# ucas-vg/PointTinyBenchmark

Hardware: AMD Instinct MI355X
Metric: img/s (640x640) CPR R50-FPN fwd+loss (higher is better)
Workload: dtype fp32

## Files before the change

include/cpr_hip.h:

```cpp
#ifndef CPR_HIP_H
#define CPR_HIP_H
#ifdef __cplusplus
extern "C" {
#endif

#define CPR_ERR_ARG (-1001)
#define CPR_ERR_UNSUPPORTED (-1002)

int cpr_version(void);

#define CPR_CONV_RELU 1
#define CPR_CONV_OUT_BF16 2
#define CPR_CONV_RES_MASK 4
#define CPR_CONV_COLSUM 8
int cpr_conv2d_fwd(const float* in, const float* wgt, float* out, const float* scale, const float* bias,
                   const float* residual, const float* in_a, const float* in_b, float* gn_part, int N, int H, int W,
                   int Cin, int Cout, int KH, int KW, int stride, int pad, int Kpad, int flags, int in_relu,
                   int* variant_out, void* stream);
int cpr_conv2d_fwd_dil(const float* in, const float* wgt, float* out, const float* scale, const float* bias,
                       const float* residual, const float* in_a, const float* in_b, float* gn_part, int N, int H, int W,
                       int Cin, int Cout, int KH, int KW, int stride, int pad, int dil, int Kpad, int flags, int in_relu,
                       int* variant_out, void* stream);

int cpr_conv2d_dual_fwd(const float* in, const float* wgt, const float* in2, const float* wgt2, float* out,
// ... 316 lines not shown
int cpr_bn_sync_bwd_merge(const double* records, int R, const double* count, const float* dout, const float* z, const float* y,
                          const float* center, const float* mean, const float* rstd, const float* gamma, float* dy, float* ws, long long M,
                          int C, void* stream);
int cpr_p2p_out_bf16_fwd(const void* x, const float* a, const float* b, const float* w, const float* bias, float* taps, float* out,
                         int N, int H, int W, int Cin, int J, void* stream);
int cpr_p2p_out_bf16_dgrad(const float* dout, int ldd, const float* w, void* dx, int out_bf16, int N, int H, int W, int Cin, int J,
                           void* stream);
int cpr_p2p_out_bf16_wgrad_ws(int N, int H, int W, int Cin, int J);
int cpr_p2p_out_bf16_wgrad(const void* x, const float* a, const float* b, const float* dout, int ldd, float* gw, float* gb, float* ws,
                           int N, int H, int W, int Cin, int J, void* stream);
int cpr_bn_fold_multi(const void* jobs_dev, int n, int max_c, void* stream);
int cpr_pack_weights_multi(const void* jobs_dev, int n, int total_blocks, void* stream);
int cpr_pack_weights_bf16_multi(const void* jobs_dev, int n, int total_blocks, void* stream);
int cpr_p2p_loss_bwd(const float* logits, const float* pred, const long long* gt_inds, const float* gt_pts,
                     const int* gt_labels, const int* gt_start, const float* npos, float* dcls, float* dreg, int B, int M,
                     int C, int Cp, int Rp, float alpha, float gamma, float beta, float pos_w, float neg_w, float reg_norm,
                     float w_cls, float w_reg, float gamma_p, const float* upstream, int cls_mode, int reg_mode, void* stream);
int cpr_p2p_loss_bwd_levels(const float* logits, const float* pred, const long long* gt_inds, const float* gt_pts,
                            const int* gt_labels, const int* gt_start, const float* npos, int B, int M, int C, int P, int L,
                            const int* level_hw, const int* level_off, const int* level_cp, const int* level_rp,
                            float* const* level_dcls, float* const* level_dreg, float alpha, float gamma, float beta, float pos_w,
                            float neg_w, float reg_norm, float w_cls, float w_reg, float gamma_p, const float* upstream,
                            int cls_mode, int reg_mode, void* stream);
int cpr_grad_sumsq(const float* g, long long n, double* ws_partial, double* out, int accumulate, void* stream);
int cpr_sgd_step(float* p, const float* grad, float* buf, const double* norm2, long long n, float lr, float mu, float wd,
                 float max_norm, float grad_scale, int first, void* stream);
int cpr_adam_step(float* p, const float* grad, float* exp_avg, float* exp_avg_sq, const double* norm2, long long n, double lr,
                  double beta1, double beta2, double eps, double wd, float step_size, float bc2_sqrt, float max_norm,
                  float grad_scale, int decoupled, void* stream);

int cpr_preprocess_u8(const unsigned char* img, const int* flip, const float* mean3, const float* stdinv3, int to_rgb,
                      float* out, int N, int H, int W, int Hp, int Wp, void* stream);
int cpr_clip_flip_boxes(float* boxes, const int* img_of, const int* flip, const int* img_hw, int n, int clip,
                        void* stream);

typedef struct cpr_preprocess_job {
    const unsigned char* src;
    long long out_off;
    double scale_x, scale_y;
    int pitch, src_w, src_h, x0, y0, cw, ch, dw, dh, flip, Hp, Wp;
} cpr_preprocess_job;
int cpr_preprocess_jobs_u8(const void* jobs_dev, int n_jobs, const float* mean3, const float* stdinv3, int to_rgb, float* out,
                           long long total_out_pixels, void* stream);
int cpr_scale_clip_flip_boxes(float* boxes, const int* img_of, const int* flip, const int* img_hw, const float* scale4, int n,
                              int clip, void* stream);

#ifdef CPR_BENCH_HOOKS
int cpr_conv_force_tile(int bm, int bn);
int cpr_conv_set_pipeline(int mode);
int cpr_conv_set_stream(int on);
int cpr_conv_set_ablation(int mode);
int cpr_wgrad_set_ablation(int mode);
int cpr_conv_set_extra_lds(int bytes);
int cpr_wino_set_variant(int sched, int ablate);
int cpr_bf16_set_dma(int on);
int cpr_bf16_set_wfrag(int on);
int cpr_wino_set_staging(int var, int tpx);
int cpr_wino32_set_debug(int ablate, int wg_per_cu, int stagger_pct);
int cpr_lsa_phase_clocks(long long* host_out, int reset);
int cpr_bn_set_finalize_only(int on);
#endif

#ifdef __cplusplus
}
#endif
#endif
```

pointtinybenchmark_amd/_lib.py:

```python
import ctypes
import os

_HERE = os.path.dirname(os.path.abspath(__file__))
LIB_PATH = os.path.join(_HERE, 'csrc', 'libcprhip.so')

_p = ctypes.c_void_p
_i = ctypes.c_int
_f = ctypes.c_float
_l = ctypes.c_longlong
_d = ctypes.c_double

SIGNATURES = {
    'cpr_version': [],
    'cpr_conv2d_fwd': [_p, _p, _p, _p, _p, _p, _p, _p, _p, _i, _i, _i, _i, _i, _i, _i, _i, _i, _i, _i, _i, _p, _p],
    'cpr_conv2d_fwd_dil': [_p] * 9 + [_i] * 13 + [_p, _p],
    'cpr_conv2d_dual_fwd': [_p] * 9 + [_i] * 16 + [_p, _p],
    'cpr_conv1x1_stream_fwd': [_p, _p, _p, _p, _p, _p, _l, _i, _i, _i, _p],
    'cpr_conv_wgrad_bf16_workspace_s': [_i] * 9,
    'cpr_conv_wgrad_bf16_s': [_p, _i, _p, _i, _p, _p] + [_i] * 8 + [_p],
    'cpr_wino_pack_weights': [_p, _p, _i, _i, _i, _p],
    'cpr_conv3x3_wino_fwd': [_p, _p, _p, _p, _p, _p, _p, _p, _i, _i, _i, _i, _i, _i, _i, _i, _p],
    'cpr_wino32_pack_weights': [_p, _p, _i, _i, _i, _p],
    'cpr_conv3x3_wino32_slots': [_i, _i],
    'cpr_conv3x3_wino32_fwd': [_p, _p, _p, _p, _p, _p, _p, _p, _i, _i, _i, _i, _i, _i, _i, _i, _p],
# ... 116 lines not shown
    'cpr_res2_conv_wgrad': [_p, _i, _i, _p, _i, _i, _p, _i, _i, _p, _p] + [_i] * 6 + [_p],
    'cpr_res2_pool_fwd': [_p, _i, _i, _p, _i, _i] + [_i] * 5 + [_p],
    'cpr_res2_relu_bwd_colsum': [_p, _i, _i, _p, _i, _i, _p, _i, _i, _p, _p, _l, _i, _p],
    'cpr_res2_pool_bwd': [_p, _i, _i, _p, _i, _i] + [_i] * 5 + [_p],
    'cpr_splat_chunks': [_i] * 3,
    'cpr_splat_gap': [_p, _p, _p] + [_i] * 4 + [_p],
    'cpr_splat_attn': [_p] * 9 + [_i] * 3 + [_p],
    'cpr_splat_apply': [_p] * 3 + [_i] * 5 + [_p],
    'cpr_splat_attn_grad': [_p] * 4 + [_i] * 5 + [_p],
    'cpr_splat_attn_bwd': [_p] * 18 + [_i] * 3 + [_p],
    'cpr_splat_apply_bwd': [_p] * 7 + [_i] * 5 + [_p],
    'cpr_dw3x3_pack': [_p, _p, _p, _i, _p],
    'cpr_dw3x3_fwd': [_p] * 5 + [_i] * 6 + [_p],
    'cpr_dw3x3_dgrad_workspace': [_i] * 4,
    'cpr_dw3x3_dgrad': [_p] * 7 + [_i] * 5 + [_p],
    'cpr_dw3x3_wgrad_workspace': [_i] * 5,
    'cpr_dw3x3_wgrad': [_p] * 4 + [_i] * 7 + [_p],
    'cpr_relu6_bwd_colsum_ws': [_l, _i],
    'cpr_relu6_bwd_colsum': [_p] * 6 + [_l, _i, _p],
    'cpr_clamp6': [_p, _l, _p],
    'cpr_spin': [ctypes.c_longlong, _p],
    'cpr_bn_fold': [_p, _p, _p, _p, _f, _p, _p, _p, _i, _p],
    'cpr_bn_train_ws': [_l, _i],
    'cpr_bn_batch_stats': [_p] * 6 + [_f, _f] + [_p] * 8 + [_l, _i, _p],
    'cpr_bn_apply': [_p] * 10 + [_l, _i, _i, _p],
    'cpr_bn_train_bwd': [_p] * 11 + [_l, _i, _p],
    'cpr_bn_sync_ws': [_l, _i],
    'cpr_bn_sync_stats_local': [_p, _p, _p, _l, _i, _p],
    'cpr_bn_sync_stats_merge': [_p, _i] + [_p] * 6 + [_f, _f] + [_p] * 8 + [_i, _p],
    'cpr_bn_sync_bwd_local': [_p] * 10 + [_l, _i, _p],
    'cpr_bn_sync_bwd_merge': [_p, _i] + [_p] * 10 + [_l, _i, _p],
    'cpr_p2p_out_bf16_fwd': [_p] * 7 + [_i] * 5 + [_p],
    'cpr_p2p_out_bf16_dgrad': [_p, _i, _p, _p] + [_i] * 6 + [_p],
    'cpr_p2p_out_bf16_wgrad_ws': [_i] * 5,
    'cpr_p2p_out_bf16_wgrad': [_p] * 4 + [_i] + [_p] * 3 + [_i] * 5 + [_p],
    'cpr_p2p_loss_bwd': [_p] * 9 + [_i] * 5 + [_f] * 9 + [_p, _i, _i, _p],
    'cpr_p2p_loss_bwd_levels': [_p] * 7 + [_i] * 5 + [_p] * 6 + [_f] * 9 + [_p, _i, _i, _p],
    'cpr_grad_sumsq': [_p, _l, _p, _p, _i, _p],
    'cpr_sgd_step': [_p, _p, _p, _p, _l, _f, _f, _f, _f, _f, _i, _p],
    'cpr_adam_step': [_p, _p, _p, _p, _p, _l, _d, _d, _d, _d, _d, _f, _f, _f, _f, _i, _p],
}

BENCH_SIGNATURES = {
    'cpr_lsa_phase_clocks': [_p, _i],
    'cpr_wino32_set_debug': [_i, _i, _i],
    'cpr_conv_force_tile': [_i, _i],
    'cpr_conv_set_pipeline': [_i],
    'cpr_conv_set_stream': [_i],
    'cpr_conv_set_ablation': [_i],
    'cpr_wgrad_set_ablation': [_i],
    'cpr_wino_set_variant': [_i, _i],
    'cpr_wino_set_staging': [_i, _i],
    'cpr_conv_set_extra_lds': [_i],
    'cpr_bf16_set_dma': [_i],
    'cpr_bf16_set_wfrag': [_i],
    'cpr_bn_set_finalize_only': [_i],
}
BENCH_LIB_PATH = os.path.join(_HERE, 'csrc', 'libcprhip_bench.so')

_lib = None


class CprHipError(RuntimeError):
    pass


def load():
    global _lib
    if _lib is not None:
        return _lib
    path, sigs = LIB_PATH, dict(SIGNATURES)
    if os.environ.get('CPR_BENCH_HOOKS', '0') == '1':
        path = BENCH_LIB_PATH
        sigs.update(BENCH_SIGNATURES)
    if not os.path.exists(path):
        raise CprHipError('%s not found: run `python -m pointtinybenchmark_amd.build%s` (no CPU fallback exists)'
                          % (path, ' --bench-hooks' if path == BENCH_LIB_PATH else ''))
    lib = ctypes.CDLL(path)
    for name, argtypes in sigs.items():
        fn = getattr(lib, name, None)
        if fn is None:
            raise CprHipError('symbol %s missing from %s (stale build?)' % (name, path))
        fn.argtypes = argtypes
        fn.restype = ctypes.c_int
    _lib = lib
    return lib


def call(name, *args, positive=False):
    rc = getattr(load(), name)(*args)
    if positive and rc >= 0:
        return rc
    if rc != 0:
        if rc == -1001:
            raise CprHipError('%s: invalid argument' % name)
        if rc == -1002:
            raise CprHipError('%s: unsupported configuration' % name)
        raise CprHipError('%s failed with hipError %d' % (name, -rc))
    return rc
```

pointtinybenchmark_amd/csrc/conv_mfma.hip:

```cpp
#include <type_traits>
#include "common.h"

struct ConvParams {
    const float* in;
    const float* wgt;
    float* out;
    const float* scale;
    const float* bias;
    const float* residual;
    const float* in_a;
    const float* in_b;
    float* gn_part;
    int N, H, W, Cin, OH, OW, Cout, KH, KW, stride, pad, Kpad, M, relu, in_relu, out_bf16;
    int res_mask;
    int tilesM, tilesN;
    const float* in2;
    const float* wgt2;
    const float* scale2;
    const float* bias2;
    int H2, W2, Cin2, stride2, Kpad2;
    int dil;
};

constexpr int BK = 32;
constexpr int LDSW = 36;

template <int BM, int BN, int MODE, bool XF, int PIPE, int ABL = 0, bool DUAL = false, bool DIL = false>
__global__ __launch_bounds__(256, 2) void conv_mfma_kernel(ConvParams p) {
    static_assert(!DUAL || (MODE == 0 && !XF && PIPE == 1 && ABL == 0), "the dual-source form exists for the plain pipelined instances");
    static_assert(!DIL || (MODE == 0 && !XF && PIPE == 1 && ABL == 0 && !DUAL), "the dilated form exists for the plain pipelined instances");
    constexpr int WM = BM / 2;
    constexpr int WN = BN / 2;
    constexpr int MI = WM / 32;
    constexpr int NI = WN / 32;
    constexpr int AL = BM * 8 / 256;
    constexpr int BL = BN * 8 / 256;
    constexpr int XFMAX = 512;
    __shared__ __attribute__((aligned(16))) float smem[2 * (BM + BN) * LDSW + (XF ? 2 * XFMAX : 0)];
    float* As = smem;
    float* Bs = smem + 2 * BM * LDSW;
    float* ABs = smem + 2 * (BM + BN) * LDSW;

    const int T = p.tilesM * p.tilesN;
    const int per = (T + 7) >> 3;
    const int tile = (blockIdx.x & 7) * per + (blockIdx.x >> 3);
    if (tile >= T) return;
    const int tm = tile / p.tilesN, tn = tile - tm * p.tilesN;
    const int m0 = tm * BM, n0 = tn * BN;

    const int tid = threadIdx.x, lane = tid & 63, wave = tid >> 6;
    const int c4 = tid & 7, r0 = tid >> 3;

    int iy0[AL], ix0[AL], nimg[AL], rowoff[AL];
    bool mok[AL];
    const int ohw = p.OH * p.OW;
    const bool gemm = (p.KH == 1) & (p.KW == 1) & (p.stride == 1) & (p.pad == 0) & (MODE == 0);
#pragma unroll
    for (int j = 0; j < AL; ++j) {
        int m = m0 + r0 + 32 * j;
        mok[j] = m < p.M;
        int mm = mok[j] ? m : 0;
        if (gemm) {
            nimg[j] = 0; iy0[j] = 0; ix0[j] = 0;
            rowoff[j] = mm * p.Cin + c4 * 4;
        } else {
            int n = mm / ohw;
            int rem = mm - n * ohw;
            int oy = rem / p.OW, ox = rem - oy * p.OW;
            nimg[j] = n;
            iy0[j] = oy * p.stride - p.pad;
            ix0[j] = ox * p.stride - p.pad;
            rowoff[j] = ((n * p.H + iy0[j]) * p.W + ix0[j]) * p.Cin + c4 * 4;
        }
    }
    __amdgpu_buffer_rsrc_t rs_in = __builtin_amdgcn_make_buffer_rsrc(
        const_cast<float*>(p.in), 0, (int)((size_t)p.N * p.H * p.W * p.Cin * 4), 0x00020000);
    __amdgpu_buffer_rsrc_t rs_w = __builtin_amdgcn_make_buffer_rsrc(
        const_cast<float*>(p.wgt), 0, (int)((size_t)p.Cout * p.Kpad * 4), 0x00020000);
    int cin_cur = p.Cin;
    bool second = false;
    const float* wrow[BL];
    int woff[BL];
    bool wok[BL];
#pragma unroll
    for (int j = 0; j < BL; ++j) {
        int c = n0 + r0 + 32 * j;
        wok[j] = c < p.Cout;
        wrow[j] = p.wgt + (size_t)(wok[j] ? c : 0) * p.Kpad + c4 * 4;
        woff[j] = wok[j] ? (c * p.Kpad + c4 * 4) * 4 : -1;
    }

    constexpr int NSET = (!XF && BM == 64 && BN == 64) ? 2 : 1;
    f32x4 ra[NSET][AL], rb[NSET][BL], xa, xb;
    unsigned okmask = 0;
    bool any_pad = true;
    int tapoff = 0;
    int kh = 0, kw = 0, c0 = 0;
    constexpr bool xform = XF;
    const float relu_floor = p.in_relu ? 0.f : -INFINITY;
    const int nblk = (m0 < p.M ? m0 : 0) / ohw;
    if (XF) {
        for (int i = tid; i < p.Cin; i += 256) {
            ABs[i] = p.in_a[nblk * p.Cin + i];
            ABs[XFMAX + i] = p.in_b[nblk * p.Cin + i];
        }
        __syncthreads();
    }

    int voffA[AL];
    unsigned okcur = 0;
    auto refresh_rows = [&]() {
        okcur = 0;
        const int dl = DIL ? p.dil : 1;
        const int tapshift = (kh * dl * p.W + kw * dl) * p.Cin;
#pragma unroll
        for (int j = 0; j < AL; ++j) {
            const int iy = iy0[j] + kh * dl, ix = ix0[j] + kw * dl;
            const bool ok = mok[j] & ((unsigned)iy < (unsigned)p.H) & ((unsigned)ix < (unsigned)p.W);
            okcur |= (ok ? 1u : 0u) << j;
            voffA[j] = ok ? (rowoff[j] + tapshift) * 4 : -1;
        }
    };
    if (MODE == 0) refresh_rows();
    auto load_a = [&](auto set_c, int kt, int j) {
        constexpr int SET = decltype(set_c)::value;
        if (MODE == 0) {
            if (j == 0) {
                okmask = okcur;
                tapoff = c0 * 4;
            }
            ra[SET][j] = __builtin_bit_cast(f32x4, __builtin_amdgcn_raw_buffer_load_b128(rs_in, voffA[j], tapoff, 0));
        } else {
            if (j == 0) okmask = 0;
            const int tap = kt * 8 + c4;
            const int th = (p.KW == 7) ? tap / 7 : tap / p.KW;
            const int tw = tap - th * p.KW;
            const int iy = iy0[j] + th, ix = ix0[j] + tw;
            const bool ok = (tap < p.KH * p.KW) & mok[j] & ((unsigned)iy < (unsigned)p.H) & ((unsigned)ix < (unsigned)p.W);
            okmask |= (ok ? 1u : 0u) << j;
            const int voff = ok ? ((nimg[j] * p.H + iy) * p.W + ix) * 16 : -1;
            ra[SET][j] = __builtin_bit_cast(f32x4, __builtin_amdgcn_raw_buffer_load_b128(rs_in, voff, 0, 0));
        }
    };
    auto load_x_advance = [&]() {
        if (MODE == 0) {
            if (xform) {
                xa = *reinterpret_cast<const f32x4*>(ABs + c0 + c4 * 4);
                xb = *reinterpret_cast<const f32x4*>(ABs + XFMAX + c0 + c4 * 4);
            }
            c0 += BK;
            if (c0 == cin_cur) {
                c0 = 0;
                if (!(DUAL && second)) {
                    if (++kw == p.KW) { kw = 0; ++kh; }
                    refresh_rows();
                }
            }
        }
    };
    int kt_last = p.Kpad / BK - 1;
    auto load_b = [&](auto set_c, int kt, int j) {
        constexpr int SET = decltype(set_c)::value;
        rb[SET][j] = __builtin_bit_cast(f32x4, __builtin_amdgcn_raw_buffer_load_b128(rs_w, woff[j], min(kt, kt_last) * (BK * 4), 0));
    };
    auto store_a = [&](auto set_c, int buf, int j) {
        constexpr int SET = decltype(set_c)::value;
        f32x4 v = ra[SET][j];
        if (MODE == 0 && xform) {
            v = v * xa + xb;
            v.x = fmaxf(v.x, relu_floor); v.y = fmaxf(v.y, relu_floor);
            v.z = fmaxf(v.z, relu_floor); v.w = fmaxf(v.w, relu_floor);
        }
        if (MODE == 0 && xform) {
            if (j == 0) any_pad = __builtin_amdgcn_ballot_w64(okmask != ((1u << AL) - 1u)) != 0;
            if (any_pad) {
                if (!((okmask >> j) & 1u)) v = f32x4{0.f, 0.f, 0.f, 0.f};
            }
        }
        *reinterpret_cast<f32x4*>(As + buf * BM * LDSW + (r0 + 32 * j) * LDSW + c4 * 4) = v;
    };
    auto store_b = [&](auto set_c, int buf, int j) {
        constexpr int SET = decltype(set_c)::value;
        *reinterpret_cast<f32x4*>(Bs + buf * BN * LDSW + (r0 + 32 * j) * LDSW + c4 * 4) = rb[SET][j];
    };
    auto load_tile = [&](auto set_c, int kt) {
#pragma unroll
        for (int j = 0; j < AL; ++j) load_a(set_c, kt, j);
        load_x_advance();
#pragma unroll
        for (int j = 0; j < BL; ++j) load_b(set_c, kt, j);
    };
    auto store_tile = [&](auto set_c, int buf) {
#pragma unroll
        for (int j = 0; j < AL; ++j) store_a(set_c, buf, j);
#pragma unroll
        for (int j = 0; j < BL; ++j) store_b(set_c, buf, j);
    };
    using Set0 = std::integral_constant<int, 0>;
    using Set1 = std::integral_constant<int, NSET - 1>;

    f32x16 acc[MI][NI];
#pragma unroll
    for (int i = 0; i < MI; ++i)
#pragma unroll
        for (int j = 0; j < NI; ++j)
#pragma unroll
            for (int r = 0; r < 16; ++r) acc[i][j][r] = 0.f;

    f32x16 acc2[DUAL ? MI : 1][DUAL ? NI : 1];
    if (DUAL) {
#pragma unroll
        for (int i = 0; i < MI; ++i)
#pragma unroll
            for (int j = 0; j < NI; ++j)
#pragma unroll
                for (int r = 0; r < 16; ++r) acc2[DUAL ? i : 0][DUAL ? j : 0][r] = 0.f;
    }

    const int wm = wave & 1, wn = wave >> 1;
    const int arow = wm * WM + (lane & 31);
    const int brow = wn * WN + (lane & 31);
    const int koff = 4 * (lane >> 5);

    int KT = p.Kpad / BK;
    const float* a_lds = As + arow * LDSW + koff;
    const float* b_lds = Bs + brow * LDSW + koff;
    auto read_frags = [&](int buf, int kk, f32x4 (&fa)[MI], f32x4 (&fb)[NI]) {
#pragma unroll
        for (int i = 0; i < MI; ++i)
            fa[i] = *reinterpret_cast<const f32x4*>(a_lds + buf * BM * LDSW + i * 32 * LDSW + kk * 8);
#pragma unroll
        for (int j = 0; j < NI; ++j)
            fb[j] = *reinterpret_cast<const f32x4*>(b_lds + buf * BN * LDSW + j * 32 * LDSW + kk * 8);
    };
    auto mfma_group = [&](const f32x4 (&fa)[MI], const f32x4 (&fb)[NI]) {
#pragma unroll
        for (int t = 0; t < 4; ++t)
#pragma unroll
            for (int i = 0; i < MI; ++i)
#pragma unroll
                for (int j = 0; j < NI; ++j)
                    acc[i][j] = __builtin_amdgcn_mfma_f32_32x32x2f32(fa[i][t], fb[j][t], acc[i][j], 0, 0, 0);
    };

    if (PIPE == 0) {
        load_tile(Set0{}, 0);
        store_tile(Set0{}, 0);
        __syncthreads();
        for (int kt = 0; kt < KT; ++kt) {
            const int buf = kt & 1;
            if (kt + 1 < KT) load_tile(Set0{}, kt + 1);
#pragma unroll
            for (int kk = 0; kk < 4; ++kk) {
                f32x4 fa[MI], fb[NI];
                read_frags(buf, kk, fa, fb);
                mfma_group(fa, fb);
            }
            if (kt + 1 < KT) store_tile(Set0{}, buf ^ 1);
            __syncthreads();
        }
    } else {
      auto kloop = [&](f32x16 (&accX)[MI][NI]) {
        f32x4 fa0[MI], fb0[NI], fa1[MI], fb1[NI];
        load_tile(Set0{}, 0);
        store_tile(Set0{}, 0);
        load_tile(Set1{}, 1);
        if (NSET == 2) load_tile(Set0{}, 2);
        __syncthreads();
        read_frags(0, 0, fa0, fb0);
        constexpr int NM = 4 * MI * NI;
        constexpr int NF = MI + NI;
        constexpr int P1 = NF + AL + BL, P2 = NF + AL + 1 + BL;
        constexpr int PPF = (NF + NM - 1) / NM, PP1 = (P1 + NM - 1) / NM, PP2 = (P2 + NM - 1) / NM;
#define MFMA_SLOT(FA, FB, q)                                                                                  \
    accX[((q) / NI) % MI][(q) % NI] = __builtin_amdgcn_mfma_f32_32x32x2f32(                                 \
        FA[((q) / NI) % MI][(q) / (MI * NI)], FB[(q) % NI][(q) / (MI * NI)], accX[((q) / NI) % MI][(q) % NI], 0, 0, 0)
#define FRAG_PIECE(FA, FB, buf, kk, z)                                                                        \
    do {                                                                                                      \
        if ((z) < MI)                                                                                         \
            FA[(z) < MI ? (z) : 0] = *reinterpret_cast<const f32x4*>(a_lds + (buf) * BM * LDSW +              \
                                                                     ((z) < MI ? (z) : 0) * 32 * LDSW + (kk) * 8); \
        else                                                                                                  \
            FB[(z) >= MI ? (z) - MI : 0] = *reinterpret_cast<const f32x4*>(                                   \
                b_lds + (buf) * BN * LDSW + ((z) >= MI ? (z) - MI : 0) * 32 * LDSW + (kk) * 8);                \
    } while (0)
        auto iteration = [&](auto nxt_c, int kt) {
            const int buf = kt & 1;
#pragma unroll
            for (int q = 0; q < NM; ++q) {
                MFMA_SLOT(fa0, fb0, q);
#pragma unroll
                for (int z = q * PPF; z < (q + 1) * PPF; ++z)
                    if (z < NF && !(ABL & 2)) FRAG_PIECE(fa1, fb1, buf, 1, z);
                __builtin_amdgcn_sched_barrier(0);
            }
#pragma unroll
            for (int q = 0; q < NM; ++q) {
                MFMA_SLOT(fa1, fb1, q);
#pragma unroll
                for (int z = q * PP1; z < (q + 1) * PP1; ++z) {
                    if (z < NF) { if (!(ABL & 2)) FRAG_PIECE(fa0, fb0, buf, 2, z); }
                    else if (ABL & 1) {}
                    else if (ABL & 8) {
                        if (z < NF + AL) asm volatile("" ::"v"(ra[decltype(nxt_c)::value][z - NF < AL ? z - NF : 0]));
                        else if (z < P1) asm volatile("" ::"v"(rb[decltype(nxt_c)::value][z - NF - AL < BL ? z - NF - AL : 0]));
                    }
                    else if (z < NF + AL) store_a(nxt_c, buf ^ 1, z - NF);
                    else if (z < P1) store_b(nxt_c, buf ^ 1, z - NF - AL);
                }
                __builtin_amdgcn_sched_barrier(0);
            }
#pragma unroll
            for (int q = 0; q < NM; ++q) {
                MFMA_SLOT(fa0, fb0, q);
#pragma unroll
                for (int z = q * PP2; z < (q + 1) * PP2; ++z) {
                    if (z < NF) { if (!(ABL & 2)) FRAG_PIECE(fa1, fb1, buf, 3, z); }
// ... 2 lines not shown
                    else if (z == NF + AL) load_x_advance();
                    else if (z < P2) load_b(nxt_c, kt + 1 + NSET, z - NF - AL - 1);
                }
                __builtin_amdgcn_sched_barrier(0);
            }
            asm volatile("" ::: "memory");
            __builtin_amdgcn_s_waitcnt(0xc07f);
            if (!(ABL & 4)) __builtin_amdgcn_s_barrier();
            asm volatile("" ::: "memory");
            __builtin_amdgcn_sched_barrier(0);
#pragma unroll
            for (int q = 0; q < NM; ++q) {
                MFMA_SLOT(fa1, fb1, q);
#pragma unroll
                for (int z = q * PPF; z < (q + 1) * PPF; ++z)
                    if (z < NF && !(ABL & 2)) FRAG_PIECE(fa0, fb0, buf ^ 1, 0, z);
                __builtin_amdgcn_sched_barrier(0);
            }
        };
        if constexpr (NSET == 2) {
            for (int kt = 0; kt < KT; kt += 2) {
                iteration(Set1{}, kt);
                if (kt + 1 < KT) iteration(Set0{}, kt + 1);
            }
        } else {
            for (int kt = 0; kt < KT; ++kt) iteration(Set0{}, kt);
        }
#undef MFMA_SLOT
#undef FRAG_PIECE
      };
      kloop(acc);
      if constexpr (DUAL) {
        rs_in = __builtin_amdgcn_make_buffer_rsrc(const_cast<float*>(p.in2), 0,
                                                  (int)((size_t)p.N * p.H2 * p.W2 * p.Cin2 * 4), 0x00020000);
        rs_w = __builtin_amdgcn_make_buffer_rsrc(const_cast<float*>(p.wgt2), 0, (int)((size_t)p.Cout * p.Kpad2 * 4), 0x00020000);
        okcur = 0;
#pragma unroll
        for (int j = 0; j < AL; ++j) {
            const int mm = mok[j] ? m0 + r0 + 32 * j : 0;
            const int n = mm / ohw;
            const int rem = mm - n * ohw;
            const int oy = rem / p.OW, ox = rem - oy * p.OW;
            okcur |= (mok[j] ? 1u : 0u) << j;
            voffA[j] = mok[j] ? (((n * p.H2 + oy * p.stride2) * p.W2 + ox * p.stride2) * p.Cin2 + c4 * 4) * 4 : -1;
        }
#pragma unroll
        for (int j = 0; j < BL; ++j) woff[j] = wok[j] ? ((n0 + r0 + 32 * j) * p.Kpad2 + c4 * 4) * 4 : -1;
        cin_cur = p.Cin2; second = true;
        kh = 0; kw = 0; c0 = 0;
        KT = p.Kpad2 / BK; kt_last = KT - 1;
        kloop(acc2);
      }
    }

    const int half = lane >> 5;
    const unsigned row_bytes = (unsigned)p.Cout * 4u;
    const __amdgpu_buffer_rsrc_t rs_out = __builtin_amdgcn_make_buffer_rsrc(
        p.out, 0, (int)((size_t)p.M * p.Cout * 4), 0x00020000);
    const __amdgpu_buffer_rsrc_t rs_res = __builtin_amdgcn_make_buffer_rsrc(
        const_cast<float*>(p.residual ? p.residual : p.out), 0, (int)((size_t)p.M * p.Cout * 4), 0x00020000);
#pragma unroll
    for (int j = 0; j < NI; ++j) {
        const int c = n0 + wn * WN + j * 32 + (lane & 31);
        const bool cok = c < p.Cout;
        const int cc = cok ? c : p.Cout - 1;
        const float sc = p.scale ? p.scale[cc] : 1.f;
        const float bi = p.bias ? p.bias[cc] : 0.f;
        const float sc2 = (DUAL && p.scale2) ? p.scale2[cc] : 1.f;
        const float bi2 = (DUAL && p.bias2) ? p.bias2[cc] : 0.f;
        float gsum = 0.f, gsq = 0.f;
#pragma unroll
        for (int i = 0; i < MI; ++i) {
            const int rbase = m0 + wm * WM + i * 32 + 4 * half;
            const unsigned off0 = cok ? (unsigned)(rbase * p.Cout + c) * 4u : 0x80000000u;
            float res[16];
            if (p.residual) {
#pragma unroll
                for (int r = 0; r < 16; ++r)
                    res[r] = __builtin_bit_cast(float, __builtin_amdgcn_raw_buffer_load_b32(
                        rs_res, (int)(off0 + (unsigned)((r & 3) + 8 * (r >> 2)) * row_bytes), 0, 0));
            } else {
#pragma unroll
                for (int r = 0; r < 16; ++r) res[r] = 0.f;
            }
#pragma unroll
            for (int r = 0; r < 16; ++r) {
                const int m = rbase + (r & 3) + 8 * (r >> 2);
                float v = acc[i][j][r] * sc + bi;
                if (DUAL) {
                    const float idv = acc2[DUAL ? i : 0][DUAL ? j : 0][r] * sc2 + bi2;
                    v += idv;
                } else if (p.res_mask) v = res[r] > 0.f ? v : 0.f;
                else v += res[r];
                if (p.relu) v = fmaxf(v, 0.f);
                if (p.out_bf16) {
                    if (cok && m < p.M) {
                        const __bf16 hv = (__bf16)v;
                        reinterpret_cast<unsigned short*>(p.out)[(size_t)m * p.Cout + c] = __builtin_bit_cast(unsigned short, hv);
                    }
                } else {
                    __builtin_amdgcn_raw_buffer_store_b32(__builtin_bit_cast(unsigned, v), rs_out,
                                                          (int)(off0 + (unsigned)((r & 3) + 8 * (r >> 2)) * row_bytes), 0, 0);
                }
                if (p.gn_part) {
                    const float u = (cok && m < p.M) ? v : 0.f;
                    gsum += u;
                    gsq += u * u;
                }
            }
        }
        if (p.gn_part) {
            gsum += __shfl_xor(gsum, 32, 64);
            gsq += __shfl_xor(gsq, 32, 64);
            const int cl = wn * WN + j * 32 + (lane & 31);
            if (half == 0) {
                smem[(wm * BN + cl) * 2 + 0] = gsum;
                smem[(wm * BN + cl) * 2 + 1] = gsq;
            }
        }
    }
    if (p.gn_part) {
        __syncthreads();
        if (tid < BN) {
            const int c = n0 + tid;
            if (c < p.Cout) {
                float s = smem[tid * 2] + smem[(BN + tid) * 2];
                float q = smem[tid * 2 + 1] + smem[(BN + tid) * 2 + 1];
                p.gn_part[((size_t)tm * p.Cout + c) * 2 + 0] = s;
                p.gn_part[((size_t)tm * p.Cout + c) * 2 + 1] = q;
            }
        }
    }
}

#ifdef CPR_BENCH_HOOKS
static int force_tile_bm = 0, force_tile_bn = 0;
static int conv_stream_on = 1;
static int conv_pipeline = 1;
static int conv_ablate = 0;
static int conv_extra_lds = 0;

extern "C" int cpr_conv_set_extra_lds(int bytes) {
    CPR_CHECK_ARG(bytes >= 0 && bytes <= 65536);
    conv_extra_lds = bytes;
    return CPR_OK;
}
extern "C" int cpr_conv_set_ablation(int mode) {
    CPR_CHECK_ARG(mode >= 0 && mode <= 16);
    conv_ablate = mode;
    return CPR_OK;
}
extern "C" int cpr_conv_set_stream(int on) {
    CPR_CHECK_ARG(on == 0 || on == 1);
    conv_stream_on = on;
    return CPR_OK;
}
extern "C" int cpr_conv_set_pipeline(int mode) {
    CPR_CHECK_ARG(mode == 0 || mode == 1);
    conv_pipeline = mode;
    return CPR_OK;
}
extern "C" int cpr_conv_force_tile(int bm, int bn) {
    CPR_CHECK_ARG((bm == 0 || bm == 64 || bm == 128) && (bn == 0 || bn == 64 || bn == 128));
    force_tile_bm = bm;
    force_tile_bn = bn;
    return CPR_OK;
}
#else
constexpr int force_tile_bm = 0, force_tile_bn = 0, conv_pipeline = 1, conv_ablate = 0, conv_extra_lds = 0, conv_stream_on = 1;
#endif

int conv1x1_stream_launch(const float* in, const float* wgt, float* out, const float* scale, const float* bias,
                          const float* residual, long long M, int Cin, int Cout, int relu, int res_mask, int min_tiles,
                          hipStream_t stream);
constexpr int STREAM_MIN_TILES = 1024;

static int conv2d_fwd_launch(const float* in, const float* wgt, float* out, const float* scale, const float* bias,
                             const float* residual, const float* in_a, const float* in_b, float* gn_part, int N,
                             int H, int W, int Cin, int Cout, int KH, int KW, int stride, int pad, int Kpad,
                             int flags, int in_relu, int bm_fix, int* variant_out, hipStream_t stream, int dil = 1) {
    CPR_CHECK_ARG(in && wgt && out);
    CPR_CHECK_ARG(dil >= 1);
    CPR_CHECK_ARG(N > 0 && H > 0 && W > 0 && Cin > 0 && Cout > 0 && KH > 0 && KW > 0 && stride > 0 && pad >= 0);
    CPR_CHECK_ARG(Kpad % BK == 0);
    ConvParams p;
    p.in = in; p.wgt = wgt; p.out = out; p.scale = scale; p.bias = bias; p.residual = residual;
    p.in_a = in_a; p.in_b = in_b; p.gn_part = gn_part;
    p.N = N; p.H = H; p.W = W; p.Cin = Cin; p.Cout = Cout; p.KH = KH; p.KW = KW; p.stride = stride; p.pad = pad;
    CPR_CHECK_ARG((flags & ~15) == 0);
    p.Kpad = Kpad; p.relu = flags & CPR_CONV_RELU; p.in_relu = in_relu; p.out_bf16 = (flags & CPR_CONV_OUT_BF16) ? 1 : 0;
    p.res_mask = (flags & CPR_CONV_RES_MASK) ? 1 : 0;
    p.in2 = nullptr; p.wgt2 = nullptr; p.scale2 = nullptr; p.bias2 = nullptr; p.H2 = p.W2 = p.Cin2 = p.stride2 = p.Kpad2 = 0;
    p.dil = dil;
    if (dil > 1)
        CPR_CHECK_ARG(KH == 3 && KW == 3 && stride == 1 && pad == dil && Cin % BK == 0 && !in_a && !in_b &&
                      (!gn_part || (flags & CPR_CONV_COLSUM)) && !(flags & CPR_CONV_OUT_BF16));
    const bool colsum_mode = (flags & CPR_CONV_COLSUM) != 0;
    if (p.res_mask) CPR_CHECK_ARG(residual != nullptr);
    p.OH = (H + 2 * pad - dil * (KH - 1) - 1) / stride + 1;
    p.OW = (W + 2 * pad - dil * (KW - 1) - 1) / stride + 1;
    CPR_CHECK_ARG(p.OH > 0 && p.OW > 0);
    long long M = (long long)N * p.OH * p.OW;
    if ((long long)N * H * W * Cin * 4 >= (1ll << 31) || (long long)Cout * Kpad * 4 >= (1ll << 31) || M >= (1ll << 31) ||
        M * Cout * 4 >= (1ll << 31))
        return CPR_ERR_UNSUPPORTED;
    p.M = (int)M;
    const bool mode1 = (Cin == 4);
    if (!mode1) {
        CPR_CHECK_ARG(Cin % BK == 0 && Kpad == KH * KW * Cin);
    } else {
        CPR_CHECK_ARG(Kpad >= KH * KW * 4 && in_a == nullptr);
    }
    if ((gn_part && !colsum_mode) || in_a) CPR_CHECK_ARG((p.OH * p.OW) % 128 == 0);
    if (in_a) CPR_CHECK_ARG(in_b && p.OH == H && p.OW == W && Cin <= 512);
    if (conv_stream_on && !mode1 && KH == 1 && KW == 1 && stride == 1 && pad == 0 && !in_a && !gn_part && !p.out_bf16 &&
        !force_tile_bm && !conv_ablate) {
        const int rc = conv1x1_stream_launch(in, wgt, out, scale, bias, residual, M, Cin, Cout, p.relu, p.res_mask,
                                             STREAM_MIN_TILES, stream);
        if (rc != CPR_ERR_UNSUPPORTED) {
            if (variant_out) *variant_out = (Cin == 256 ? 128 : 8192 / Cin) * 1000000 + (Cin == 256 ? 64 : 16384 / Cin) * 1000 + 3;
            return rc;
        }
    }
    int bm = 128, bn = (Cout <= 64) ? 64 : 128;
    if ((!gn_part || colsum_mode) && !in_a && !mode1) {
        const long long t128 = (long long)((p.M + 127) / 128) * ((Cout + 127) / 128);
        const int kt = Kpad / BK;
        if (!(kt >= 16 && t128 >= 4096 && Cout > 64)) { bm = 64; bn = 64; }
    }
    if (force_tile_bm > 0 && (!gn_part || colsum_mode) && !in_a && !mode1) { bm = force_tile_bm; }
    if (bm_fix > 0) bm = bm_fix;
    if (force_tile_bn > 0 && Cout > 64 && !mode1) { bn = force_tile_bn; }
    if (variant_out) *variant_out = bm * 1000000 + bn * 1000 + (mode1 ? 100 : 0) + (in_a ? 10 : 0) + conv_pipeline;
    p.tilesM = (p.M + bm - 1) / bm;
    p.tilesN = (Cout + bn - 1) / bn;
    const int T = p.tilesM * p.tilesN;
    const int grid = ((T + 7) / 8) * 8;
#ifdef CPR_BENCH_HOOKS
#define LAUNCH(BM_, BN_, MODE_, XF_)                                                                               \
    do {                                                                                                           \
        if (conv_pipeline == 0)                                                                                    \
            hipLaunchKernelGGL((conv_mfma_kernel<BM_, BN_, MODE_, XF_, 0>), dim3(grid), dim3(256), conv_extra_lds, stream, p); \
        else                                                                                                       \
            hipLaunchKernelGGL((conv_mfma_kernel<BM_, BN_, MODE_, XF_, 1>), dim3(grid), dim3(256), conv_extra_lds, stream, p); \
    } while (0)
#else
#define LAUNCH(BM_, BN_, MODE_, XF_) \
    hipLaunchKernelGGL((conv_mfma_kernel<BM_, BN_, MODE_, XF_, 1>), dim3(grid), dim3(256), 0, stream, p)
#endif
#ifdef CPR_BENCH_HOOKS
    if (conv_ablate && !mode1 && !in_a && bm == 128 && bn == 128) {
        switch (conv_ablate) {
            case 1: hipLaunchKernelGGL((conv_mfma_kernel<128, 128, 0, false, 1, 1>), dim3(grid), dim3(256), 0, stream, p); break;
            case 2: hipLaunchKernelGGL((conv_mfma_kernel<128, 128, 0, false, 1, 2>), dim3(grid), dim3(256), 0, stream, p); break;
            case 3: hipLaunchKernelGGL((conv_mfma_kernel<128, 128, 0, false, 1, 3>), dim3(grid), dim3(256), 0, stream, p); break;
            case 4: hipLaunchKernelGGL((conv_mfma_kernel<128, 128, 0, false, 1, 4>), dim3(grid), dim3(256), 0, stream, p); break;
            case 8: hipLaunchKernelGGL((conv_mfma_kernel<128, 128, 0, false, 1, 8>), dim3(grid), dim3(256), 0, stream, p); break;
            case 16: hipLaunchKernelGGL((conv_mfma_kernel<128, 128, 0, false, 1, 16>), dim3(grid), dim3(256), 0, stream, p); break;
            default: hipLaunchKernelGGL((conv_mfma_kernel<128, 128, 0, false, 1, 7>), dim3(grid), dim3(256), 0, stream, p); break;
        }
    } else
#endif
    if (dil > 1) {
#define LAUNCH_DIL(BM_, BN_) \
    hipLaunchKernelGGL((conv_mfma_kernel<BM_, BN_, 0, false, 1, 0, false, true>), dim3(grid), dim3(256), 0, stream, p)
        if (bm == 128) { if (bn == 64) LAUNCH_DIL(128, 64); else LAUNCH_DIL(128, 128); }
        else { if (bn == 64) LAUNCH_DIL(64, 64); else LAUNCH_DIL(64, 128); }
#undef LAUNCH_DIL
    } else if (mode1) {
        if (bn == 64) LAUNCH(128, 64, 1, false); else LAUNCH(128, 128, 1, false);
    } else if (in_a) {
        if (bn == 64) LAUNCH(128, 64, 0, true); else LAUNCH(128, 128, 0, true);
    } else if (bm == 128) {
        if (bn == 64) LAUNCH(128, 64, 0, false); else LAUNCH(128, 128, 0, false);
    } else {
        if (bn == 64) LAUNCH(64, 64, 0, false); else LAUNCH(64, 128, 0, false);
    }
#undef LAUNCH
    CPR_LAUNCH_STATUS();
}

extern "C" int cpr_conv2d_fwd(const float* in, const float* wgt, float* out, const float* scale, const float* bias,
                              const float* residual, const float* in_a, const float* in_b, float* gn_part, int N,
                              int H, int W, int Cin, int Cout, int KH, int KW, int stride, int pad, int Kpad,
                              int flags, int in_relu, int* variant_out, hipStream_t stream) {
    CPR_CHECK_ARG(N > 0 && H > 0 && W > 0 && Cin > 0 && Cout > 0 && KH > 0 && KW > 0 && stride > 0 && pad >= 0);
    const int OH = (H + 2 * pad - KH) / stride + 1, OW = (W + 2 * pad - KW) / stride + 1;
    CPR_CHECK_ARG(OH > 0 && OW > 0);
    const long long in_img = (long long)H * W * Cin * 4, out_img = (long long)OH * OW * Cout * ((flags & CPR_CONV_OUT_BF16) ? 2 : 4);
    const long long res_img = (long long)OH * OW * Cout * 4;
    int align = 1;
    if (flags & CPR_CONV_COLSUM) { const long long r = (long long)OH * OW; align = 1; while ((r * align) % 128 != 0) align *= 2; }
    const int per = cpr_images_per_launch(N, cpr_max2(cpr_max2(in_img, out_img), residual ? res_img : 0), align);
    if (per <= 0) return CPR_ERR_UNSUPPORTED;
    if (per >= N) return conv2d_fwd_launch(in, wgt, out, scale, bias, residual, in_a, in_b, gn_part, N, H, W, Cin, Cout, KH, KW,
                                           stride, pad, Kpad, flags, in_relu, 0, variant_out, stream);
    int bm_fix = 0, variant = 0;
    const size_t oe = (flags & CPR_CONV_OUT_BF16) ? 2 : 4;
    for (int n0 = 0; n0 < N; n0 += per) {
        const int n = N - n0 < per ? N - n0 : per;
        const size_t rows = (size_t)n0 * OH * OW;
        float* part = nullptr;
        if (gn_part) part = gn_part + ((flags & CPR_CONV_COLSUM) ? (bm_fix ? rows / bm_fix : 0) : rows / 128) * Cout * 2;
        const int rc = conv2d_fwd_launch(in + (size_t)n0 * H * W * Cin, wgt, (float*)((char*)out + rows * Cout * oe), scale, bias,
                                         residual ? residual + rows * Cout : nullptr, in_a ? in_a + (size_t)n0 * Cin : nullptr,
                                         in_b ? in_b + (size_t)n0 * Cin : nullptr, part, n, H, W, Cin, Cout, KH, KW, stride, pad,
                                         Kpad, flags, in_relu, bm_fix, &variant, stream);
        if (rc != CPR_OK) return rc;
        if (n0 == 0) { if (flags & CPR_CONV_COLSUM) bm_fix = variant / 1000000; if (variant_out) *variant_out = variant; }
    }
    return CPR_OK;
}

extern "C" int cpr_conv2d_fwd_dil(const float* in, const float* wgt, float* out, const float* scale, const float* bias,
                                  const float* residual, const float* in_a, const float* in_b, float* gn_part, int N, int H,
                                  int W, int Cin, int Cout, int KH, int KW, int stride, int pad, int dil, int Kpad, int flags,
                                  int in_relu, int* variant_out, hipStream_t stream) {
    CPR_CHECK_ARG(dil >= 1);
    if (dil == 1)
        return cpr_conv2d_fwd(in, wgt, out, scale, bias, residual, in_a, in_b, gn_part, N, H, W, Cin, Cout, KH, KW, stride, pad, Kpad,
                              flags, in_relu, variant_out, stream);
    CPR_CHECK_ARG(in && wgt && out && N > 0 && H > 0 && W > 0 && Cin > 0 && Cout > 0);
    CPR_CHECK_ARG(KH == 3 && KW == 3 && stride == 1 && pad == dil && Cin % BK == 0 && Kpad == 9 * Cin);
    CPR_CHECK_ARG(!in_a && !in_b && in_relu == 0 && (flags & ~15) == 0 && !(flags & CPR_CONV_OUT_BF16));
    CPR_CHECK_ARG(!gn_part == !(flags & CPR_CONV_COLSUM));
    if ((flags & CPR_CONV_RES_MASK)) CPR_CHECK_ARG(residual != nullptr);
    const long long img = (long long)H * W * (Cin > Cout ? Cin : Cout) * 4;
    int align = 1;
    if (flags & CPR_CONV_COLSUM) { const long long r = (long long)H * W; while ((r * align) % 128 != 0) align *= 2; }
    const int per = cpr_images_per_launch(N, img, align);
    if (per <= 0) return CPR_ERR_UNSUPPORTED;
    int bm_fix = 0, variant = 0;
    for (int n0 = 0; n0 < N; n0 += per) {
        const int n = N - n0 < per ? N - n0 : per;
        const size_t rows = (size_t)n0 * H * W;
        float* part = gn_part ? gn_part + (bm_fix ? rows / bm_fix : 0) * Cout * 2 : nullptr;
        const int rc = conv2d_fwd_launch(in + rows * Cin, wgt, out + rows * Cout, scale, bias, residual ? residual + rows * Cout : nullptr,
                                         nullptr, nullptr, part, n, H, W, Cin, Cout, 3, 3, 1, pad, Kpad, flags, 0, bm_fix, &variant,
                                         stream, dil);
        if (rc != CPR_OK) return rc;
        if (n0 == 0) { if (flags & CPR_CONV_COLSUM) bm_fix = variant / 1000000; if (variant_out) *variant_out = variant; }
    }
    return CPR_OK;
}

static int conv2d_dual_launch(const float* in, const float* wgt, const float* in2, const float* wgt2, float* out,
                              const float* scale, const float* bias, const float* scale2, const float* bias2, int N, int H,
                              int W, int Cin, int Cout, int KH, int KW, int stride, int pad, int Kpad, int H2, int W2,
                              int Cin2, int stride2, int Kpad2, int flags, int* variant_out, hipStream_t stream) {
    ConvParams p;
    p.in = in; p.wgt = wgt; p.out = out; p.scale = scale; p.bias = bias; p.residual = nullptr;
    p.in_a = nullptr; p.in_b = nullptr; p.gn_part = nullptr;
    p.N = N; p.H = H; p.W = W; p.Cin = Cin; p.Cout = Cout; p.KH = KH; p.KW = KW; p.stride = stride; p.pad = pad;
    p.Kpad = Kpad; p.relu = flags & CPR_CONV_RELU; p.in_relu = 0; p.out_bf16 = 0; p.res_mask = 0;
    p.OH = (H + 2 * pad - KH) / stride + 1;
    p.OW = (W + 2 * pad - KW) / stride + 1;
    p.in2 = in2; p.wgt2 = wgt2; p.scale2 = scale2; p.bias2 = bias2;
    p.H2 = H2; p.W2 = W2; p.Cin2 = Cin2; p.stride2 = stride2; p.Kpad2 = Kpad2;
    p.tilesM = p.tilesN = 0;
    const long long M = (long long)N * p.OH * p.OW;
    if ((long long)N * H * W * Cin * 4 >= (1ll << 31) || (long long)N * H2 * W2 * Cin2 * 4 >= (1ll << 31) ||
        (long long)Cout * Kpad * 4 >= (1ll << 31) || (long long)Cout * Kpad2 * 4 >= (1ll << 31) || M * Cout * 4 >= (1ll << 31))
        return CPR_ERR_UNSUPPORTED;
    p.M = (int)M;
    int bm = 64, bn = 64;
    const long long t128 = (long long)((p.M + 127) / 128) * ((Cout + 127) / 128);
    if ((Kpad + Kpad2) / BK >= 16 && t128 >= 4096 && Cout > 64) { bm = 128; bn = 128; }
    if (force_tile_bm > 0) { bm = bn = force_tile_bm; }
    if (variant_out) *variant_out = bm * 1000000 + bn * 1000 + 2;
    p.tilesM = (p.M + bm - 1) / bm;
    p.tilesN = (Cout + bn - 1) / bn;
    const int grid = ((p.tilesM * p.tilesN + 7) / 8) * 8;
    if (bm == 64) hipLaunchKernelGGL((conv_mfma_kernel<64, 64, 0, false, 1, 0, true>), dim3(grid), dim3(256), 0, stream, p);
    else hipLaunchKernelGGL((conv_mfma_kernel<128, 128, 0, false, 1, 0, true>), dim3(grid), dim3(256), 0, stream, p);
    CPR_LAUNCH_STATUS();
}

extern "C" int cpr_conv2d_dual_fwd(const float* in, const float* wgt, const float* in2, const float* wgt2, float* out,
                                   const float* scale, const float* bias, const float* scale2, const float* bias2, int N,
                                   int H, int W, int Cin, int Cout, int KH, int KW, int stride, int pad, int Kpad, int H2,
                                   int W2, int Cin2, int stride2, int Kpad2, int flags, int* variant_out, hipStream_t stream) {
    CPR_CHECK_ARG(in && wgt && in2 && wgt2 && out);
    CPR_CHECK_ARG(N > 0 && H > 0 && W > 0 && Cin > 0 && Cout > 0 && KH > 0 && KW > 0 && stride > 0 && pad >= 0);
    CPR_CHECK_ARG(H2 > 0 && W2 > 0 && Cin2 > 0 && stride2 > 0 && (flags & ~CPR_CONV_RELU) == 0);
    CPR_CHECK_ARG(Cin % BK == 0 && Kpad == KH * KW * Cin && Cin2 % BK == 0 && Kpad2 == Cin2);
    const int OH = (H + 2 * pad - KH) / stride + 1, OW = (W + 2 * pad - KW) / stride + 1;
    CPR_CHECK_ARG(OH > 0 && OW > 0 && OH == (H2 - 1) / stride2 + 1 && OW == (W2 - 1) / stride2 + 1);
    const long long img = cpr_max2(cpr_max2((long long)H * W * Cin, (long long)H2 * W2 * Cin2), (long long)OH * OW * Cout) * 4;
    const int per = cpr_images_per_launch(N, img);
    if (per <= 0) return CPR_ERR_UNSUPPORTED;
    for (int n0 = 0; n0 < N; n0 += per) {
        const int n = N - n0 < per ? N - n0 : per;
        const int rc = conv2d_dual_launch(in + (size_t)n0 * H * W * Cin, wgt, in2 + (size_t)n0 * H2 * W2 * Cin2, wgt2,
                                          out + (size_t)n0 * OH * OW * Cout, scale, bias, scale2, bias2, n, H, W, Cin, Cout,
                                          KH, KW, stride, pad, Kpad, H2, W2, Cin2, stride2, Kpad2, flags,
                                          n0 == 0 ? variant_out : nullptr, stream);
        if (rc != CPR_OK) return rc;
    }
    return CPR_OK;
}
```

Measured before the change: 914.2.

## Make 128x128 conv MFMA kernel persistent with next-tile head prefetch

Adds a persistent-tile variant of the 128x128 implicit-GEMM conv kernel. The grid is capped at two workgroups per CU, and each workgroup loops over tiles. It issues the first K-slice loads of the next tile before the current tile's epilogue, so that load latency overlaps the stores. This is meant to remove per-workgroup launch and ramp-up cost and tail effects on large convs. The cost is a loop-carried setup, an extra barrier per tile, and possible imbalance from the strided tile assignment.

```diff
diff --git a/include/cpr_hip.h b/include/cpr_hip.h
--- a/include/cpr_hip.h
+++ b/include/cpr_hip.h
@@ -392,6 +392,7 @@
 int cpr_conv_set_ablation(int mode);
 int cpr_wgrad_set_ablation(int mode);
 int cpr_conv_set_extra_lds(int bytes);
+int cpr_conv_set_one_tile(int on);
 int cpr_wino_set_variant(int sched, int ablate);
 int cpr_bf16_set_dma(int on);
 int cpr_bf16_set_wfrag(int on);
diff --git a/pointtinybenchmark_amd/_lib.py b/pointtinybenchmark_amd/_lib.py
--- a/pointtinybenchmark_amd/_lib.py
+++ b/pointtinybenchmark_amd/_lib.py
@@ -192,6 +192,7 @@
     'cpr_wino_set_variant': [_i, _i],
     'cpr_wino_set_staging': [_i, _i],
     'cpr_conv_set_extra_lds': [_i],
+    'cpr_conv_set_one_tile': [_i],
     'cpr_bf16_set_dma': [_i],
     'cpr_bf16_set_wfrag': [_i],
     'cpr_bn_set_finalize_only': [_i],
diff --git a/pointtinybenchmark_amd/csrc/conv_mfma.hip b/pointtinybenchmark_amd/csrc/conv_mfma.hip
--- a/pointtinybenchmark_amd/csrc/conv_mfma.hip
+++ b/pointtinybenchmark_amd/csrc/conv_mfma.hip
@@ -25,10 +25,12 @@
 constexpr int BK = 32;
 constexpr int LDSW = 36;
 
-template <int BM, int BN, int MODE, bool XF, int PIPE, int ABL = 0, bool DUAL = false, bool DIL = false>
+template <int BM, int BN, int MODE, bool XF, int PIPE, int ABL = 0, bool DUAL = false, bool DIL = false, bool PERSIST = false>
 __global__ __launch_bounds__(256, 2) void conv_mfma_kernel(ConvParams p) {
     static_assert(!DUAL || (MODE == 0 && !XF && PIPE == 1 && ABL == 0), "the dual-source form exists for the plain pipelined instances");
     static_assert(!DIL || (MODE == 0 && !XF && PIPE == 1 && ABL == 0 && !DUAL), "the dilated form exists for the plain pipelined instances");
+    static_assert(!PERSIST || (BM == 128 && BN == 128 && MODE == 0 && PIPE == 1 && ABL == 0 && !DUAL && !DIL),
+                  "the persistent tile loop exists for the instances it was measured to help");
     constexpr int WM = BM / 2;
     constexpr int WN = BN / 2;
     constexpr int MI = WM / 32;
@@ -43,10 +45,10 @@
 
     const int T = p.tilesM * p.tilesN;
     const int per = (T + 7) >> 3;
-    const int tile = (blockIdx.x & 7) * per + (blockIdx.x >> 3);
+    int vb = blockIdx.x;
+    int tile = (vb & 7) * per + (vb >> 3);
     if (tile >= T) return;
-    const int tm = tile / p.tilesN, tn = tile - tm * p.tilesN;
-    const int m0 = tm * BM, n0 = tn * BN;
+    int tm = 0, m0 = 0, n0 = 0;
 
     const int tid = threadIdx.x, lane = tid & 63, wave = tid >> 6;
     const int c4 = tid & 7, r0 = tid >> 3;
@@ -55,40 +57,14 @@
     bool mok[AL];
     const int ohw = p.OH * p.OW;
     const bool gemm = (p.KH == 1) & (p.KW == 1) & (p.stride == 1) & (p.pad == 0) & (MODE == 0);
-#pragma unroll
-    for (int j = 0; j < AL; ++j) {
-        int m = m0 + r0 + 32 * j;
-        mok[j] = m < p.M;
-        int mm = mok[j] ? m : 0;
-        if (gemm) {
-            nimg[j] = 0; iy0[j] = 0; ix0[j] = 0;
-            rowoff[j] = mm * p.Cin + c4 * 4;
-        } else {
-            int n = mm / ohw;
-            int rem = mm - n * ohw;
-            int oy = rem / p.OW, ox = rem - oy * p.OW;
-            nimg[j] = n;
-            iy0[j] = oy * p.stride - p.pad;
-            ix0[j] = ox * p.stride - p.pad;
-            rowoff[j] = ((n * p.H + iy0[j]) * p.W + ix0[j]) * p.Cin + c4 * 4;
-        }
-    }
     __amdgpu_buffer_rsrc_t rs_in = __builtin_amdgcn_make_buffer_rsrc(
         const_cast<float*>(p.in), 0, (int)((size_t)p.N * p.H * p.W * p.Cin * 4), 0x00020000);
     __amdgpu_buffer_rsrc_t rs_w = __builtin_amdgcn_make_buffer_rsrc(
         const_cast<float*>(p.wgt), 0, (int)((size_t)p.Cout * p.Kpad * 4), 0x00020000);
     int cin_cur = p.Cin;
     bool second = false;
-    const float* wrow[BL];
     int woff[BL];
     bool wok[BL];
-#pragma unroll
-    for (int j = 0; j < BL; ++j) {
-        int c = n0 + r0 + 32 * j;
-        wok[j] = c < p.Cout;
-        wrow[j] = p.wgt + (size_t)(wok[j] ? c : 0) * p.Kpad + c4 * 4;
-        woff[j] = wok[j] ? (c * p.Kpad + c4 * 4) * 4 : -1;
-    }
 
     constexpr int NSET = (!XF && BM == 64 && BN == 64) ? 2 : 1;
     f32x4 ra[NSET][AL], rb[NSET][BL], xa, xb;
@@ -98,14 +74,7 @@
     int kh = 0, kw = 0, c0 = 0;
     constexpr bool xform = XF;
     const float relu_floor = p.in_relu ? 0.f : -INFINITY;
-    const int nblk = (m0 < p.M ? m0 : 0) / ohw;
-    if (XF) {
-        for (int i = tid; i < p.Cin; i += 256) {
-            ABs[i] = p.in_a[nblk * p.Cin + i];
-            ABs[XFMAX + i] = p.in_b[nblk * p.Cin + i];
-        }
-        __syncthreads();
-    }
+    int nblk_lds = -1;
 
     int voffA[AL];
     unsigned okcur = 0;
@@ -121,7 +90,49 @@
             voffA[j] = ok ? (rowoff[j] + tapshift) * 4 : -1;
         }
     };
-    if (MODE == 0) refresh_rows();
+    int KT = p.Kpad / BK, kt_last = KT - 1;
+    auto setup_tile = [&](int t) {
+        tm = t / p.tilesN;
+        const int tn = t - tm * p.tilesN;
+        m0 = tm * BM; n0 = tn * BN;
+#pragma unroll
+        for (int j = 0; j < AL; ++j) {
+            int m = m0 + r0 + 32 * j;
+            mok[j] = m < p.M;
+            int mm = mok[j] ? m : 0;
+            if (gemm) {
+                nimg[j] = 0; iy0[j] = 0; ix0[j] = 0;
+                rowoff[j] = mm * p.Cin + c4 * 4;
+            } else {
+                int n = mm / ohw;
+                int rem = mm - n * ohw;
+                int oy = rem / p.OW, ox = rem - oy * p.OW;
+                nimg[j] = n;
+                iy0[j] = oy * p.stride - p.pad;
+                ix0[j] = ox * p.stride - p.pad;
+                rowoff[j] = ((n * p.H + iy0[j]) * p.W + ix0[j]) * p.Cin + c4 * 4;
+            }
+        }
+#pragma unroll
+        for (int j = 0; j < BL; ++j) {
+            int c = n0 + r0 + 32 * j;
+            wok[j] = c < p.Cout;
+            woff[j] = wok[j] ? (c * p.Kpad + c4 * 4) * 4 : -1;
+        }
+        if (XF) {
+            const int nblk = (m0 < p.M ? m0 : 0) / ohw;
+            if (nblk != nblk_lds) {
+                nblk_lds = nblk;
+                for (int i = tid; i < p.Cin; i += 256) {
+                    ABs[i] = p.in_a[nblk * p.Cin + i];
+                    ABs[XFMAX + i] = p.in_b[nblk * p.Cin + i];
+                }
+                __syncthreads();
+            }
+        }
+        kh = 0; kw = 0; c0 = 0;
+        if (MODE == 0) refresh_rows();
+    };
     auto load_a = [&](auto set_c, int kt, int j) {
         constexpr int SET = decltype(set_c)::value;
         if (MODE == 0) {
@@ -158,7 +169,6 @@
             }
         }
     };
-    int kt_last = p.Kpad / BK - 1;
     auto load_b = [&](auto set_c, int kt, int j) {
         constexpr int SET = decltype(set_c)::value;
         rb[SET][j] = __builtin_bit_cast(f32x4, __builtin_amdgcn_raw_buffer_load_b128(rs_w, woff[j], min(kt, kt_last) * (BK * 4), 0));
@@ -199,30 +209,32 @@
     using Set0 = std::integral_constant<int, 0>;
     using Set1 = std::integral_constant<int, NSET - 1>;
 
+    auto request_head = [&]() { load_tile(Set0{}, 0); };
+
     f32x16 acc[MI][NI];
-#pragma unroll
-    for (int i = 0; i < MI; ++i)
-#pragma unroll
-        for (int j = 0; j < NI; ++j)
-#pragma unroll
-            for (int r = 0; r < 16; ++r) acc[i][j][r] = 0.f;
-
     f32x16 acc2[DUAL ? MI : 1][DUAL ? NI : 1];
-    if (DUAL) {
+    auto zero_acc = [&]() {
 #pragma unroll
         for (int i = 0; i < MI; ++i)
 #pragma unroll
             for (int j = 0; j < NI; ++j)
 #pragma unroll
-                for (int r = 0; r < 16; ++r) acc2[DUAL ? i : 0][DUAL ? j : 0][r] = 0.f;
-    }
+                for (int r = 0; r < 16; ++r) acc[i][j][r] = 0.f;
+        if (DUAL) {
+#pragma unroll
+            for (int i = 0; i < MI; ++i)
+#pragma unroll
+                for (int j = 0; j < NI; ++j)
+#pragma unroll
+                    for (int r = 0; r < 16; ++r) acc2[DUAL ? i : 0][DUAL ? j : 0][r] = 0.f;
+        }
+    };
 
     const int wm = wave & 1, wn = wave >> 1;
     const int arow = wm * WM + (lane & 31);
     const int brow = wn * WN + (lane & 31);
     const int koff = 4 * (lane >> 5);
 
-    int KT = p.Kpad / BK;
     const float* a_lds = As + arow * LDSW + koff;
     const float* b_lds = Bs + brow * LDSW + koff;
     auto read_frags = [&](int buf, int kk, f32x4 (&fa)[MI], f32x4 (&fb)[NI]) {
@@ -243,6 +255,7 @@
                     acc[i][j] = __builtin_amdgcn_mfma_f32_32x32x2f32(fa[i][t], fb[j][t], acc[i][j], 0, 0, 0);
     };
 
+    auto run_k = [&]() {
     if (PIPE == 0) {
         load_tile(Set0{}, 0);
         store_tile(Set0{}, 0);
@@ -262,7 +275,7 @@
     } else {
       auto kloop = [&](f32x16 (&accX)[MI][NI]) {
         f32x4 fa0[MI], fb0[NI], fa1[MI], fb1[NI];
-        load_tile(Set0{}, 0);
+        if (!PERSIST) load_tile(Set0{}, 0);
         store_tile(Set0{}, 0);
         load_tile(Set1{}, 1);
         if (NSET == 2) load_tile(Set0{}, 2);
@@ -371,9 +384,28 @@
         kloop(acc2);
       }
     }
+    };
 
     const int half = lane >> 5;
     const unsigned row_bytes = (unsigned)p.Cout * 4u;
+    setup_tile(tile);
+    if (PERSIST) request_head();
+    for (;;) {
+        const int m0_cur = m0, n0_cur = n0, tm_cur = tm;
+        zero_acc();
+        run_k();
+        bool more = false;
+        if constexpr (PERSIST) {
+            vb += gridDim.x;
+            tile = (vb & 7) * per + (vb >> 3);
+            more = (vb < 8 * per) & (tile < T);
+            if (more) {
+                setup_tile(tile);
+                request_head();
+            }
+        }
+    {
+    const int m0 = m0_cur, n0 = n0_cur, tm = tm_cur;
     const __amdgpu_buffer_rsrc_t rs_out = __builtin_amdgcn_make_buffer_rsrc(
         p.out, 0, (int)((size_t)p.M * p.Cout * 4), 0x00020000);
     const __amdgpu_buffer_rsrc_t rs_res = __builtin_amdgcn_make_buffer_rsrc(
@@ -449,6 +481,10 @@
                 p.gn_part[((size_t)tm * p.Cout + c) * 2 + 1] = q;
             }
         }
+        if (PERSIST) __syncthreads();
+    }
+    }
+        if (!more) break;
     }
 }
 
@@ -458,6 +494,13 @@
 static int conv_pipeline = 1;
 static int conv_ablate = 0;
 static int conv_extra_lds = 0;
+static int conv_one_tile = 0;
+
+extern "C" int cpr_conv_set_one_tile(int on) {
+    CPR_CHECK_ARG(on == 0 || on == 1);
+    conv_one_tile = on;
+    return CPR_OK;
+}
 
 extern "C" int cpr_conv_set_extra_lds(int bytes) {
     CPR_CHECK_ARG(bytes >= 0 && bytes <= 65536);
@@ -487,7 +530,24 @@
 }
 #else
 constexpr int force_tile_bm = 0, force_tile_bn = 0, conv_pipeline = 1, conv_ablate = 0, conv_extra_lds = 0, conv_stream_on = 1;
+constexpr int conv_one_tile = 0;
 #endif
+
+static int conv_grid(int tiles, bool persist) {
+    static int cu_of_device[64] = {};
+    int dev = 0, ncu = 256;
+    if (hipGetDevice(&dev) == hipSuccess && dev >= 0 && dev < 64) {
+        if (cu_of_device[dev] == 0) {
+            int v = 0;
+            if (hipDeviceGetAttribute(&v, hipDeviceAttributeMultiprocessorCount, dev) == hipSuccess && v > 0) cu_of_device[dev] = v;
+        }
+        if (cu_of_device[dev] > 0) ncu = cu_of_device[dev];
+    }
+    ncu = (ncu + 7) / 8 * 8;
+    const int slots = ncu * 2;
+    const int grid = (tiles + 7) / 8 * 8;
+    return (persist && grid > slots) ? slots : grid;
+}
 
 int conv1x1_stream_launch(const float* in, const float* wgt, float* out, const float* scale, const float* bias,
                           const float* residual, long long M, int Cin, int Cout, int relu, int res_mask, int min_tiles,
@@ -553,8 +613,10 @@
     if (variant_out) *variant_out = bm * 1000000 + bn * 1000 + (mode1 ? 100 : 0) + (in_a ? 10 : 0) + conv_pipeline;
     p.tilesM = (p.M + bm - 1) / bm;
     p.tilesN = (Cout + bn - 1) / bn;
-    const int T = p.tilesM * p.tilesN;
-    const int grid = ((T + 7) / 8) * 8;
+    const bool persist = bm == 128 && bn == 128 && !mode1 && dil == 1 && conv_pipeline == 1 && !conv_ablate && !conv_one_tile;
+    const int grid = conv_grid(p.tilesM * p.tilesN, persist);
+#define LAUNCH_PERSIST(XF_) \
+    hipLaunchKernelGGL((conv_mfma_kernel<128, 128, 0, XF_, 1, 0, false, false, true>), dim3(grid), dim3(256), conv_extra_lds, stream, p)
 #ifdef CPR_BENCH_HOOKS
 #define LAUNCH(BM_, BN_, MODE_, XF_)                                                                               \
     do {                                                                                                           \
@@ -589,13 +651,14 @@
     } else if (mode1) {
         if (bn == 64) LAUNCH(128, 64, 1, false); else LAUNCH(128, 128, 1, false);
     } else if (in_a) {
-        if (bn == 64) LAUNCH(128, 64, 0, true); else LAUNCH(128, 128, 0, true);
+        if (bn == 64) LAUNCH(128, 64, 0, true); else if (persist) LAUNCH_PERSIST(true); else LAUNCH(128, 128, 0, true);
     } else if (bm == 128) {
-        if (bn == 64) LAUNCH(128, 64, 0, false); else LAUNCH(128, 128, 0, false);
+        if (bn == 64) LAUNCH(128, 64, 0, false); else if (persist) LAUNCH_PERSIST(false); else LAUNCH(128, 128, 0, false);
     } else {
         if (bn == 64) LAUNCH(64, 64, 0, false); else LAUNCH(64, 128, 0, false);
     }
 #undef LAUNCH
+#undef LAUNCH_PERSIST
     CPR_LAUNCH_STATUS();
 }
 
@@ -689,7 +752,7 @@
     if (variant_out) *variant_out = bm * 1000000 + bn * 1000 + 2;
     p.tilesM = (p.M + bm - 1) / bm;
     p.tilesN = (Cout + bn - 1) / bn;
-    const int grid = ((p.tilesM * p.tilesN + 7) / 8) * 8;
+    const int grid = conv_grid(p.tilesM * p.tilesN, false);
     if (bm == 64) hipLaunchKernelGGL((conv_mfma_kernel<64, 64, 0, false, 1, 0, true>), dim3(grid), dim3(256), 0, stream, p);
     else hipLaunchKernelGGL((conv_mfma_kernel<128, 128, 0, false, 1, 0, true>), dim3(grid), dim3(256), 0, stream, p);
     CPR_LAUNCH_STATUS();
```

After: 915.7, median of 5. Within noise of the previous version (+0.2%).
